# adrientremblay/Skillshot_Learning

Hardware: AMD Instinct MI355X
Metric: env-steps/sec (whole node) at 65536 self-play envs; 1/2/4/8 GPU scaling (higher is better)
Workload: dtype f64

## Files before the change

skillshot_learning_amd/csrc/sk_engine.hip:

```cpp
#include <hip/hip_runtime.h>

#include <cmath>
#include <cstdio>
#include <cstdlib>
#include <cstring>
#include <string>
#include <type_traits>
#include <vector>

#include "sk_device.hpp"
#include "sk_host.hpp"
#include "sk_range.hpp"
#include "sk_step.hpp"


using namespace sk;

struct sk_env {
  int32_t n;
  int64_t env_offset;
  uint64_t seed;
  int32_t device;
  sk_config cfg;
  Cfg dcfg;
  View view;
  sk_state_view hview;
  bool owned;
  char* d_aux;
  sk_counters* d_counters;
  uint64_t* d_step;
  int parity;
  int step_variant;
  int multi_policy;
  int multi_split;
  int multi_early;
  int multi_block;
  int multi_stagger;
  int multi_prefetch;
  int multi_pack;
  int multi_fast;
  char* d_pack;
  skh::Host* host;
};

static thread_local std::string g_err;

static int fail(int code, const std::string& msg) {
  g_err = msg;
  return code;
}

#define HIP_TRY(expr)                                                                 \
  do {                                                                                \
    hipError_t _e = (expr);                                                           \
    if (_e != hipSuccess)                                                             \
      return fail(SK_EHIP, std::string(#expr) + ": " + hipGetErrorString(_e));       \
  } while (0)

static constexpr int kBlock = 256;
static constexpr int64_t kFastStepMinEnvs = 196608;
static constexpr int64_t kFastStepMaxEnvs = 786432;
static constexpr int64_t kSplitStepMaxEnvs = 8192;
static constexpr int64_t kEarlyDrawMinEnvs = 32768;
constexpr int64_t kPackMinEnvs = 65536;
static constexpr int64_t kSplitMultiMaxEnvs = 32768;
static constexpr int64_t kSplitPackMinEnvs = 40960;
static constexpr int64_t kSplitPackMaxEnvs = 98304;
static constexpr int kFastSplitMinTicks = 100;
static constexpr int kSteadyRest = 7;
static inline int64_t counter_slots(int64_t n) {
  const int64_t w2 = (2 * n + 63) / 64, w8 = (n + 7) / 8, waves = w2 > w8 ? w2 : w8;
  return waves * SK_CTR_STRIDE > SK_COUNTER_SLOTS ? waves * SK_CTR_STRIDE : SK_COUNTER_SLOTS;
}
static inline size_t aux_bytes(int64_t n) { return 256 + (size_t)counter_slots(n) * sizeof(sk_counters); }

static inline unsigned grid_for(int64_t n) { return (unsigned)((n + kBlock - 1) / kBlock); }
static inline unsigned step_grid(int64_t n) { return (unsigned)((n + kStepBlock - 1) / kStepBlock); }

__device__ __forceinline__ float reward_of(const Cfg& c, const Env& e, int p, int kind, double path_dist) {
  if (kind == SK_REWARD_SIMPLE) {
    int o = 1 - p;
    double mine = dist_point_point(e.qx[p], e.qy[p], e.px[o], e.py[o]);
    double theirs = dist_point_point(e.qx[o], e.qy[o], e.px[p], e.py[p]);
    return (float)(mine - theirs);
  }
  return (float)(-path_dist / (double)c.W);
}

#ifdef SK_TRACE_STEP
__device__ unsigned long long* sk_step_trace;
#define SK_TS(var) const unsigned long long var = __builtin_amdgcn_s_memrealtime()
#else
#define SK_TS(var)
#endif

template <bool OBS>
__global__ void __launch_bounds__(kStepBlock) k_step(StepArgs a, Cfg c) {
  int64_t i = (int64_t)blockIdx.x * kStepBlock + threadIdx.x;
  SK_TS(ts0);
  WaveCtr wc = ctr_load(a.ctr);
  const uint64_t step = step_read(a.step);
  step_advance(a.step, step, 1);
  bool in = i < a.n;
  bool d = false;
  Env e;
  double q_old0 = 0.0, q_old1 = 0.0;
  sktrig::SinCos tq0 = {0.0, 1.0}, tq1 = {0.0, 1.0};
  U4 ru = {0u, 0u, 0u, 0u};
#ifdef SK_TRACE_STEP
  unsigned long long ts1 = 0, ts2 = 0;
#endif
  if (in) {
    load_env(a.v, i, e);
    q_old0 = e.qrot[0];
    q_old1 = e.qrot[1];
    __builtin_amdgcn_sched_barrier(0);
    const float2 a0 = load_action(a.actions + i);
    const float2 a1 = load_action(a.actions + a.n + i);
    __builtin_amdgcn_sched_barrier(0);
    if (a.random_positions && a.n >= kEarlyDrawMinEnvs) {
      ru = draw4(a.seed, (uint64_t)(a.env_offset + i), step, 1u);
      asm volatile("" : "+v"(ru.x), "+v"(ru.y), "+v"(ru.z), "+v"(ru.w));
    }
    __builtin_amdgcn_sched_barrier(0);
#ifdef SK_TRACE_STEP
    __builtin_amdgcn_s_waitcnt(0);
    ts1 = __builtin_amdgcn_s_memrealtime();
    __builtin_amdgcn_sched_barrier(0);
#endif
    bool k0, k1;
    const sktrig::SinCos m0 = sktrig::sincos_bf(e.rot[0], &k0);
    const sktrig::SinCos m1 = sktrig::sincos_bf(e.rot[1], &k1);
    tick_env_m(c, e, m0, m1, k0 & k1, (double)a0.x, (double)a0.y, (double)a1.x, (double)a1.y, OBS ? &tq0 : nullptr,
               OBS ? &tq1 : nullptr);
#ifdef SK_TRACE_STEP
    __builtin_amdgcn_sched_barrier(0);
    ts2 = __builtin_amdgcn_s_memrealtime();
    __builtin_amdgcn_sched_barrier(0);
#endif
  }
  ctr_settle(wc);
  float o0[12], o1[12];
  unsigned amb = 0;
  double g0 = 0.0, g1 = 0.0;
  if (in) {
    if (OBS && (a.obs || a.reward || a.obs_reset)) {
      float pd0, pd1;
      amb = obs_env_sc(c, e, tq0, tq1, o0, o1, &pd0, &pd1, &g0, &g1);
      if (a.obs) {
        store_obs(a.obs, a.n, 0, i, o0);
        store_obs(a.obs, a.n, 1, i, o1);
        if (amb) fix_future_flags_g(c, e, amb, g0, g1, a.obs, a.n, i);
      }
      if (a.reward) {
        a.reward[i] = reward_of(c, e, 0, a.reward_kind, (double)pd0);
        a.reward[a.n + i] = reward_of(c, e, 1, a.reward_kind, (double)pd1);
      }
    }
    d = (!e.live) || (e.ticks >= a.tick_limit);
    if (a.done) a.done[i] = (uint8_t)d;
    if (a.winner) a.winner[i] = (uint8_t)e.winner;
  }
  const int fin_winner = in ? e.winner : 0, fin_ticks = in ? e.ticks : 0;
  if (in && d && a.auto_reset) {
    if (a.random_positions) {
      if (a.n >= kEarlyDrawMinEnvs) reset_random_u(c, e, ru);
      else reset_random(c, e, a.seed, (uint64_t)(a.env_offset + i), step);
    }
    else reset_fixed(c, e);
  }
  if (OBS && in && a.obs_reset) {
    if (d && a.auto_reset) {
      float pd0, pd1;
      amb = obs_env_sc(c, e, sktrig::SinCos{0.0, 1.0}, sktrig::SinCos{0.0, 1.0}, o0, o1, &pd0, &pd1);
    }
    store_obs(a.obs_reset, a.n, 0, i, o0);
    store_obs(a.obs_reset, a.n, 1, i, o1);
    if (amb) fix_future_flags_g(c, e, amb, g0, g1, a.obs_reset, a.n, i);
  }
  if (in) store_env_q(a.v, i, e, q_old0, q_old1);
  if (a.ctr) wave_count(a.ctr, wc, d, fin_winner, fin_ticks);
  if (!in) return;
#ifdef SK_TRACE_STEP
  __builtin_amdgcn_s_waitcnt(0);
  const unsigned long long ts3 = __builtin_amdgcn_s_memrealtime();
  if ((threadIdx.x & 63) == 0 && sk_step_trace) {
    const unsigned waves = gridDim.x * (blockDim.x >> 6);
    const unsigned w = blockIdx.x * (blockDim.x >> 6) + (threadIdx.x >> 6);
    unsigned long long* t = sk_step_trace + ((step & 15) * waves + w) * 8;
    t[0] = ts0; t[1] = ts1; t[2] = ts2; t[3] = ts3;
    t[4] = __builtin_amdgcn_s_getreg((31 << 11) | 4);
    t[5] = __builtin_amdgcn_s_getreg((15 << 11) | 20);
  }
#endif
}

#ifdef SK_TRACE_STEP
extern "C" int skdiag_set_step_trace(void* buf) {
  return hipMemcpyToSymbol(HIP_SYMBOL(sk_step_trace), &buf, sizeof(buf)) == hipSuccess ? 0 : -1;
}
#endif

__global__ void __launch_bounds__(kStepBlock) k_step_fast(StepArgs a, Cfg c) {
  int64_t i = (int64_t)blockIdx.x * kStepBlock + threadIdx.x;
  bool in = i < a.n;
  StepLoads L;
  if (in) issue_step_loads(a.v, a.actions, a.n, i, L);
  WaveCtr wc = ctr_load(a.ctr);
  bool d = false;
  Env e;
  if (in) {
    wait_rot(L);
    bool k0, k1, k2, k3;
    sktrig::SinCosF m0 = sktrig::sincos_fast(L.r.x, &k0);
    sktrig::SinCosF m1 = sktrig::sincos_fast(L.r.y, &k1);
    wait_qrot(L, m0, m1);
    sktrig::SinCosF tq0 = sktrig::sincos_fast(L.qr.x, &k2);
    sktrig::SinCosF tq1 = sktrig::sincos_fast(L.qr.y, &k3);
    wait_state(L, tq0, tq1);
    decode_env(step_loads_env(L), e);
    wait_actions(L);
    tick_env_fast(c, e, m0, m1, tq0, tq1, k0 & k1, k2, k3, L.a0.x, L.a0.y, L.a1.x, L.a1.y);
// ... 499 lines not shown
      SK_MTW(t, 0);
      asm volatile("s_waitcnt vmcnt(0)" ::: "memory");
      SK_MTW(t, 1);
    }
#endif
    multi_compute<POL, PACK>(a, c, r, rp, L, wc, so, step0, t, w, packed, t + 1 == a.n_ticks, tc);
#if defined(SK_TRACE_MULTI_WAIT)
    SK_MTW(t, 4);
#elif defined(SK_TRACE_MULTI)
    if (t < 29) SK_MTS(1 + t);
#endif
    slab = slab + 1 == a.ring ? 0 : slab + 1;
    pslab = pslab + 1 == a.ring ? 0 : pslab + 1;
    so = so + 1 == a.out_slabs ? 0 : so + 1;
  };
  do {
    one_tick(pa0, pa1);
    if (++t >= a.n_ticks) break;
    one_tick(pa1, pa0);
  } while (++t < a.n_ticks);
  if (a.ctr) {
    const unsigned c4[4] = {L.n_done, L.n_h1, L.n_h2, L.t_sum};
    uint64_t v[4];
    wave_sum4_u32(c4, v);
    ctr_store<BLK>(a.ctr, wc, v[0], v[1], v[2], v[3]);
  }
  step_advance(a.step, step0, (uint64_t)a.n_ticks);
  SK_MTS(31);
}

template <int POL>
__device__ __forceinline__ void st_half_d(const MultiArgs& a, __amdgpu_buffer_rsrc_t r, int k, double* plane, int64_t h,
                                          double v) {
  if constexpr (POL == 0) plane[h] = v;
  else __builtin_amdgcn_raw_buffer_store_b64(__builtin_bit_cast(skb2i, v), r, (uint32_t)h * 8u + a.off[k], 0, 16);
}
template <int POL>
__device__ __forceinline__ void st_half_i(const MultiArgs& a, __amdgpu_buffer_rsrc_t r, int k, int2* plane, int64_t h,
                                          int x, int y) {
  if constexpr (POL == 0) plane[h] = make_int2(x, y);
  else __builtin_amdgcn_raw_buffer_store_b64((skb2i){x, y}, r, (uint32_t)h * 8u + a.off[k], 0, 16);
}
struct SplitLane {
  int64_t i, ic, hc, h;
  int p;
  bool in;
  unsigned n_done, n_h1, n_h2, t_sum;
};

struct SplitCarry {
  double kr, kq;
  sktrig::SinCos m, tq;
  double pr;
  bool qs, have, pend;
};
__device__ __forceinline__ void split_carry_advance(SplitCarry& t) {
  bool k;
  t.m = sktrig::sincos_bf(t.pr, &k);
  if (!k) t.m = sincos_lib(t.pr);
  t.kr = t.pr;
  if (t.qs) {
    t.tq = t.m;
    t.kq = t.pr;
  }
  t.have = true;
  t.pend = false;
}
struct SplitCarryF {
  double kr, kq;
  sktrig::SinCosF m;
  int dx, dy;
  double pr;
  bool mok, qex, have, pend;
};
__device__ __forceinline__ void split_carry_advance(SplitCarryF& t) {
  t.m = sktrig::sincos_fast(t.pr, &t.mok);
  t.kr = t.pr;
  t.have = true;
  t.pend = false;
}
__device__ __forceinline__ void split_carry_pin(SplitCarry& t) {
  asm volatile("" : "+v"(t.m.s), "+v"(t.m.c), "+v"(t.tq.s), "+v"(t.tq.c));
}
__device__ __forceinline__ void split_carry_pin(SplitCarryF& t) {
  asm volatile("" : "+v"(t.m.s), "+v"(t.m.c));
}
template <bool FAST>
struct SplitCarrySel {
  using type = SplitCarry;
};
template <>
struct SplitCarrySel<true> {
  using type = SplitCarryF;
};
struct SplitRaw {
  skb2i rot, qrot, pp, ca, qq, mi;
};
template <int POL>
__device__ __forceinline__ skb2i ld_half_raw(const MultiArgs& a, __amdgpu_buffer_rsrc_t r, int k, const void* plane,
                                             int64_t h) {
  if constexpr (POL == 0) return reinterpret_cast<const skb2i*>(plane)[h];
  else return __builtin_amdgcn_raw_buffer_load_b64(r, (uint32_t)h * 8u + a.off[k], 0, 16);
}
template <int POL>
__device__ __forceinline__ void split_load_raw(const MultiArgs& a, __amdgpu_buffer_rsrc_t r, const SplitLane& L,
                                               SplitRaw& w) {
  w.rot = ld_half_raw<POL>(a, r, 1, a.v.rot, L.hc);
  w.qrot = ld_half_raw<POL>(a, r, 3, a.v.qrot, L.hc);
  w.pp = ld_half_raw<POL>(a, r, 0, a.v.pos, L.hc);
  w.ca = ld_half_raw<POL>(a, r, 4, a.v.qcdage, L.hc);
  w.qq = ld_half_raw<POL>(a, r, 2, a.v.qpos, L.hc);
  w.mi = ld_half_raw<POL>(a, r, 5, a.v.misc, L.ic);
  __builtin_amdgcn_sched_barrier(0);
}
template <int POL>
__device__ __forceinline__ void split_store_state(const MultiArgs& a, __amdgpu_buffer_rsrc_t r, const SplitLane& L,
                                                  int px, int py, double rot, int qx, int qy, double qrot, bool qch,
                                                  int qcd, int qage, int ticks, unsigned f) {
  st_half_i<POL>(a, r, 0, reinterpret_cast<int2*>(a.v.pos), L.h, px, py);
  st_half_d<POL>(a, r, 1, reinterpret_cast<double*>(a.v.rot), L.h, rot);
  st_half_i<POL>(a, r, 2, reinterpret_cast<int2*>(a.v.qpos), L.h, qx, qy);
  if (qch) st_half_d<POL>(a, r, 3, reinterpret_cast<double*>(a.v.qrot), L.h, qrot);
  st_half_i<POL>(a, r, 4, reinterpret_cast<int2*>(a.v.qcdage), L.h, qcd, qage);
  if (L.p == 0) st_half_i<POL>(a, r, 5, a.v.misc, L.i, ticks, (int)f);
}
template <int POL>
__device__ __forceinline__ void split_load_pack(const MultiArgs& a, __amdgpu_buffer_rsrc_t rp, const SplitLane& L,
                                                SplitRaw& w) {
  if constexpr (POL == 0) {
    const skb2i* P = reinterpret_cast<const skb2i*>(a.pack);
    w.rot = P[L.hc];
    w.qrot = P[2 * a.n + L.hc];
    w.pp = P[4 * a.n + L.hc];
  } else {
    const uint32_t o = (uint32_t)L.hc * 8u, plane = (uint32_t)a.n * 16u;
    w.rot = __builtin_amdgcn_raw_buffer_load_b64(rp, o, 0, 16);
    w.qrot = __builtin_amdgcn_raw_buffer_load_b64(rp, o + plane, 0, 16);
    w.pp = __builtin_amdgcn_raw_buffer_load_b64(rp, o + 2u * plane, 0, 16);
  }
  __builtin_amdgcn_sched_barrier(0);
}
template <int POL>
__device__ __forceinline__ void split_store_pack(const MultiArgs& a, __amdgpu_buffer_rsrc_t rp, const SplitLane& L,
                                                 double rot, double qrot, bool store_q, int pos, int cah) {
  if constexpr (POL == 0) {
    skb2i* P = reinterpret_cast<skb2i*>(a.pack);
    P[L.h] = __builtin_bit_cast(skb2i, rot);
    if (store_q) P[2 * a.n + L.h] = __builtin_bit_cast(skb2i, qrot);
    P[4 * a.n + L.h] = (skb2i){pos, cah};
  } else {
    const uint32_t o = (uint32_t)L.h * 8u, plane = (uint32_t)a.n * 16u;
    __builtin_amdgcn_raw_buffer_store_b64(__builtin_bit_cast(skb2i, rot), rp, o, 0, 16);
    if (store_q) __builtin_amdgcn_raw_buffer_store_b64(__builtin_bit_cast(skb2i, qrot), rp, o + plane, 0, 16);
    __builtin_amdgcn_raw_buffer_store_b64((skb2i){pos, cah}, rp, o + 2u * plane, 0, 16);
  }
}
struct SplitSteady {
  __amdgpu_buffer_rsrc_t ra, rd, rw;
  uint32_t va, vd;
  uint32_t aso, dso;
};
struct SplitPre {
  float l;
  double dl;
  sktrig::SinCosF u;
  float ex, ey;
  float mdx, mdy;
  bool msafe, qsafe;
  int imx, imy, iex, iey;
};
__device__ __forceinline__ SplitPre split_fast_pre(const sktrig::SinCosF& m, bool mok, float2 act, const Cfg& c) {
  SplitPre q;
  const float qsf = (float)c.qspeed;
  q.l = clamp_action_f(act.y);
  q.dl = (double)q.l * c.look;
  q.u = sktrig::sincos_add(m, q.l * (float)c.look);
  q.ex = q.u.s * qsf;
  q.ey = q.u.c * qsf;
  const sktrig::FastDelta dm = sktrig::fast_move_delta(m, mok, (float)c.pspeed, clamp_action_f(act.x));
  q.mdx = dm.x;
  q.mdy = dm.y;
  q.msafe = dm.safe;
  q.qsafe = sktrig::fast_step_delta(q.u, mok, qsf).safe;
  q.imx = (int)rintf(q.mdx);
  q.imy = (int)rintf(q.mdy);
  q.iex = (int)rintf(q.ex);
  q.iey = (int)rintf(q.ey);
  return q;
}
__device__ __forceinline__ void split_pre_pin(SplitPre& q) {
  unsigned long long ms = __builtin_amdgcn_ballot_w64(q.msafe), qs = __builtin_amdgcn_ballot_w64(q.qsafe);
  asm volatile("" : "+v"(q.dl), "+v"(q.imx), "+v"(q.imy), "+v"(q.iex), "+v"(q.iey), "+s"(ms), "+s"(qs));
  q.msafe = __builtin_amdgcn_inverse_ballot_w64(ms);
  q.qsafe = __builtin_amdgcn_inverse_ballot_w64(qs);
}
template <int POL, bool OBS, bool PACK = false, bool FAST = false, bool STEADY = false, bool FULL = false>
__device__ __forceinline__ void split_tick_carry(const MultiArgs& a, const Cfg& c, __amdgpu_buffer_rsrc_t r,
                                                 SplitLane& L, WaveCtr& wc, int64_t so, uint64_t step,
                                                 const SplitRaw& w, float2 act,
                                                 typename SplitCarrySel<FAST>::type& tc, bool last,
                                                 __amdgpu_buffer_rsrc_t rp, bool& packed,
                                                 const SplitSteady* ss = nullptr, SplitPre* pre = nullptr,
                                                 int left = 0, bool* admit = nullptr) {
  constexpr bool PRE = FAST && STEADY;
  static_assert(!(OBS && PACK), "the full contract never packs");
  static_assert(!(OBS && FAST), "the observation needs the exact sincos");
  static_assert(PACK || !STEADY, "the steady loop is the packed kernel's");
  static_assert(STEADY || !FULL, "the full-wave form is the steady loop's");
  using sktrig::round_safe;
  const int p = L.p;
  const bool in = FULL || L.in;
  double rot = __builtin_bit_cast(double, w.rot), qrot = __builtin_bit_cast(double, w.qrot);
  int px = w.pp.x, py = w.pp.y, qx = w.qq.x, qy = w.qq.y, qcd = w.ca.x, qage = w.ca.y, ticks = w.mi.x;
  const unsigned flags = (unsigned)w.mi.y;
  int qvalid = (flags >> (8 * p)) & 0xff, live = (flags >> 16) & 0xff, winner = (flags >> 24) & 0xff;
  if constexpr (PACK) {
    if (STEADY || packed) {
      const unsigned s = (unsigned)w.pp.x, ch = (unsigned)w.pp.y;
      px = s & 0xff; py = (s >> 8) & 0xff; qx = (s >> 16) & 0xff; qy = s >> 24;
      qcd = (int)(signed char)(ch & 0xff); qage = (ch >> 8) & 0xff;
      const unsigned hi = ch >> 16, ohi = (unsigned)pair_swap((int)hi);
      const unsigned fl = p ? hi : ohi;
      ticks = (int)(p ? ohi : hi);
      qvalid = (fl >> p) & 1; live = (fl >> 2) & 1; winner = (fl >> 3) & 3;
    }
  }
  const double q_old = qrot;
  const bool f = qcd <= 0;
  const bool miss = (!STEADY && !tc.have) || !same_bits(rot, tc.kr) || (qvalid && !f && !same_bits(qrot, tc.kq));
  if (__ballot(in && miss) != 0) {
    if constexpr (FAST) {
      bool kq;
      tc.m = sktrig::sincos_fast(rot, &tc.mok);
      const sktrig::SinCosF q = sktrig::sincos_fast(qrot, &kq);
      const sktrig::FastDelta d = sktrig::fast_step_delta(q, kq, (float)c.qspeed);
      tc.qex = !d.safe;
      tc.dx = (int)rintf(d.x);
      tc.dy = (int)rintf(d.y);
    } else {
      bool k0, k1;
      tc.m = sktrig::sincos_bf(rot, &k0);
      tc.tq = sktrig::sincos_bf(qrot, &k1);
      if (!(k0 & k1)) {
        if (!k0) tc.m = sincos_lib(rot);
        if (!k1) tc.tq = sincos_lib(qrot);
      }
    }
    tc.kr = rot;
    tc.kq = qrot;
    tc.have = true;
    if constexpr (PRE) *pre = split_fast_pre(tc.m, tc.mok, act, c);
  }
  SplitPre q{};
  if constexpr (PRE) q = *pre;
  const float l = PRE ? q.l : clamp_action_f(act.y);
  const double rn = rot + (PRE ? q.dl : (double)l * c.look);
  const float lk = (float)c.look, qsf = (float)c.qspeed, eq = 2e-6f * qsf;
  sktrig::SinCosF mf;
  if constexpr (FAST) mf = tc.m;
  else mf = sktrig::SinCosF{(float)tc.m.s, (float)tc.m.c};
  const sktrig::SinCosF u = PRE ? q.u : sktrig::sincos_add(mf, l * lk);
  const float ex = PRE ? q.ex : u.s * qsf, ey = PRE ? q.ey : u.c * qsf;
  bool un, unq = false;
  float mdx = 0.0f, mdy = 0.0f;
  sktrig::SinCos tt{0.0, 1.0};
  sktrig::SinCos tm{0.0, 1.0};
  if constexpr (PRE) {
    mdx = q.mdx;
    mdy = q.mdy;
    unq = f && !q.qsafe;
    un = !q.msafe || unq || (qvalid && !f && tc.qex);
  } else if constexpr (FAST) {
    const sktrig::FastDelta dm = sktrig::fast_move_delta(tc.m, tc.mok, (float)c.pspeed, clamp_action_f(act.x));
    mdx = dm.x;
    mdy = dm.y;
    unq = f && !sktrig::fast_step_delta(u, tc.mok, qsf).safe;
    un = !dm.safe || unq || (qvalid && !f && tc.qex);
  } else {
    un = f && !((int)(fabs(rot) < 1647099.3291652855) & (int)round_safe(ex, eq) & (int)round_safe(ey, eq));
    tt = tc.tq;
    tm = tc.m;
  }
  bool fast = f;
  bool exact = false;
  int epx = 0, epy = 0, enx = 0, eny = 0;
  sktrig::SinCos xn{0.0, 1.0};
  sktrig::SinCosF pr{0.0f, 1.0f};
  if constexpr (OBS) {
    bool kx, k2;
    xn = sktrig::sincos_bf(rn, &kx);
    pr = sktrig::sincos_fast(rn, &k2);
    if (!(kx & k2)) {
      if (!kx) xn = sincos_lib(rn);
      if (!k2) {
        const sktrig::SinCos rr = sincos_lib(rn);
        pr.s = (float)rr.s;
        pr.c = (float)rr.c;
      }
    }
  }
  if (__builtin_expect(__ballot(in && un) != 0, 0)) {
    if constexpr (FAST) {
      const double qa = f ? rn : qrot;
      bool k0, k1;
      tm = sktrig::sincos_bf(rot, &k0);
      tt = sktrig::sincos_bf(qa, &k1);
      if (!(k0 & k1)) {
        if (!k0) tm = sincos_lib(rot);
        if (!k1) tt = sincos_lib(qa);
      }
      const double speed = clamp_action((double)act.x), psp = (double)c.pspeed, qsp = (double)c.qspeed;
      const double nxf = __builtin_rint((double)px - (tm.s * psp) * speed);
      const double nyf = __builtin_rint((double)py - (tm.c * psp) * speed);
      const bool ok = (nxf >= 0.0) & (nxf + (double)c.psize <= (double)c.W) & (nyf >= 0.0) &
                      (nyf + (double)c.psize <= (double)c.H);
      epx = ok ? (int)(ok ? nxf : 0.0) : px;
      epy = ok ? (int)(ok ? nyf : 0.0) : py;
      enx = (int)__builtin_rint((double)(f ? epx : qx) - tt.s * qsp);
      eny = (int)__builtin_rint((double)(f ? epy : qy) - tt.c * qsp);
      exact = true;
    } else {
      sktrig::SinCos x = xn;
      if constexpr (!OBS) {
        bool k;
        x = sktrig::sincos_bf(rn, &k);
        if (!k) x = sincos_lib(rn);
      }
      if (f) tt = x;
      fast = false;
    }
  }
  sktrig::SinCos tq_obs{0.0, 1.0};
  if constexpr (OBS) tq_obs = f ? xn : tc.tq;
  if constexpr (!FAST) {
    const double speed = clamp_action((double)act.x), psp = (double)c.pspeed;
    const double nxf = __builtin_rint((double)px - (tm.s * psp) * speed);
    const double nyf = __builtin_rint((double)py - (tm.c * psp) * speed);
    const bool ok = (nxf >= 0.0) & (nxf + (double)c.psize <= (double)c.W) & (nyf >= 0.0) &
                    (nyf + (double)c.psize <= (double)c.H);
    px = ok ? (int)(ok ? nxf : 0.0) : px;
    py = ok ? (int)(ok ? nyf : 0.0) : py;
  } else {
    const int nx = px - (PRE ? q.imx : (int)rintf(mdx)), ny = py - (PRE ? q.imy : (int)rintf(mdy));
    bool ok;
    if constexpr (STEADY) ok = skrange::fits_board(nx, ny, c.W - c.psize, c.H - c.psize);
    else ok = (nx >= 0) & (nx <= c.W - c.psize) & (ny >= 0) & (ny <= c.H - c.psize);
    px = exact ? epx : (ok ? nx : px);
    py = exact ? epy : (ok ? ny : py);
  }
  rot = rn;
  qx = f ? px : qx;
  qy = f ? py : qy;
  qrot = f ? rot : qrot;
  qvalid = f ? 1 : qvalid;
  qcd = f ? c.cdmax : qcd;
  qage = f ? 0 : qage;
  const int lv = live != 0;
  ticks += lv;
  {
    const double qsp = (double)c.qspeed;
    int nx, ny;
    if constexpr (FAST) {
      const int sdx = f ? (PRE ? q.iex : (int)rintf(ex)) : tc.dx, sdy = f ? (PRE ? q.iey : (int)rintf(ey)) : tc.dy;
      tc.dx = sdx;
      tc.dy = sdy;
      tc.qex = f ? unq : tc.qex;
      tc.kq = f ? rn : tc.kq;
      nx = exact ? enx : qx - sdx;
      ny = exact ? eny : qy - sdy;
    } else {
      const int nxF = qx - (int)rintf(ex), nyF = qy - (int)rintf(ey);
      const int nxE = (int)__builtin_rint((double)qx - tt.s * qsp), nyE = (int)__builtin_rint((double)qy - tt.c * qsp);
      nx = fast ? nxF : nxE;
      ny = fast ? nyF : nyE;
    }
    bool ok;
    if constexpr (STEADY) ok = skrange::fits_board(nx, ny, c.W - c.qsize, c.H - c.qsize);
    else ok = (nx + c.qsize <= c.W) & (nx >= 0) & (ny + c.qsize <= c.H) & (ny >= 0);
    const bool upd = lv && qvalid;
    qx = (upd && ok) ? nx : qx;
    qy = (upd && ok) ? ny : qy;
    qvalid = (upd && !ok) ? 0 : qvalid;
    qcd -= lv;
    qage += lv;
  }
  int opx = 0, opy = 0;
  if constexpr (!PACK) {
    opx = pair_swap(px);
    opy = pair_swap(py);
  }
  const int oqx = pair_swap(qx), oqy = pair_swap(qy), oqv = pair_swap(qvalid);
  if constexpr (PACK) {
    bool mine;
    if constexpr (STEADY) mine = (int)(oqv != 0) & (int)skrange::box_hit(px, py, c.psize, oqx, oqy, c.qsize);
    else mine = hit_test_s(c, px, py, oqx, oqy, oqv);
    const bool theirs = pair_swap((int)mine) != 0;
    const skrange::PairHit h = skrange::pair_hit(lv != 0, p ? theirs : mine, p ? mine : theirs);
    winner = h.h1 ? 1 : (h.h2 ? 2 : winner);
    live = ((int)h.h1 | (int)h.h2) ? 0 : live;
  } else {
    const int p1x = p ? opx : px, p1y = p ? opy : py, q1x = p ? oqx : qx, q1y = p ? oqy : qy, q1v = p ? oqv : qvalid;
    const int p2x = p ? px : opx, p2y = p ? py : opy, q2x = p ? qx : oqx, q2y = p ? qy : oqy, q2v = p ? qvalid : oqv;
    const bool h1 = lv && hit_test_s(c, p1x, p1y, q2x, q2y, q2v);
    const bool h2 = lv && !h1 && hit_test_s(c, p2x, p2y, q1x, q1y, q1v);
    winner = h1 ? 1 : (h2 ? 2 : winner);
    live = (h1 || h2) ? 0 : live;
  }
  if constexpr (!STEADY) ctr_settle(wc);
  bool to_pack = STEADY;
  if constexpr (PACK && !STEADY) {
    const bool fit = !in || ((int)pack_fits_player(px, py, qx, qy, qcd, qage, qvalid) &
                               (int)pack_fits_game(ticks, live, winner));
    to_pack = !last && __ballot(!fit) == 0;
    const bool adm = !in || ((int)skrange::admit_player(px, py, qx, qy, qcd, qage, qvalid) &
                               (int)skrange::admit_game(ticks, live, winner, left));
    *admit = to_pack && __ballot(!adm) == 0;
  }
  if (PACK && to_pack) {
    const bool qch = (!STEADY && !packed) || __double_as_longlong(qrot) != __double_as_longlong(q_old);
    const unsigned hi = p ? pack_flags(oqv, qvalid, live, winner) : (unsigned)ticks;
    if (in) split_store_pack<POL>(a, rp, L, rot, qrot, qch, pack_pos(px, py, qx, qy), pack_cah(qcd, qage, hi));
  } else {
    const unsigned fl = (unsigned)(qvalid & 0xff) | ((unsigned)(oqv & 0xff) << 8) | ((unsigned)(live & 0xff) << 16) |
                        ((unsigned)(winner & 0xff) << 24);
    const bool qch = STEADY || (PACK && packed) || __double_as_longlong(qrot) != __double_as_longlong(q_old);
    if (in) split_store_state<POL>(a, r, L, px, py, rot, qx, qy, qrot, qch, qcd, qage, ticks, fl);
  }
  bool amb = false;
  double gq = 0.0;
  const int aqx = qx, aqy = qy;
  const double aqrot = qrot;
  if constexpr (OBS) {
    if (in) {
      float o[12], pd;
      obs12_sc(c, px, py, rot, pr, qx, qy, qrot, tq_obs, qcd, qvalid, opx, opy, o, &pd, &amb, &gq);
      if (a.obs) store_obs(a.obs + so * 24 * a.n, a.n, p, L.i, o);
      if (a.reward) {
        float rw;
        if (a.reward_kind == SK_REWARD_SIMPLE) {
          const double mine = dist_point_point(qx, qy, opx, opy);
          const double theirs = dist_point_point(oqx, oqy, px, py);
          rw = (float)(mine - theirs);
        } else {
          rw = (float)(-(double)pd / (double)c.W);
        }
        a.reward[so * 2 * a.n + (int64_t)p * a.n + L.i] = rw;
      }
    }
  }
  const bool d = in && ((!live) || (ticks >= a.tick_limit));
  if (in && p == 0) {
    if constexpr (STEADY) {
      __builtin_amdgcn_raw_buffer_store_b8((unsigned char)d, ss->rd, ss->vd, ss->dso, 0);
      __builtin_amdgcn_raw_buffer_store_b8((unsigned char)winner, ss->rw, ss->vd, ss->dso, 0);
    } else {
      if (a.done) a.done[so * a.out_stride + L.i] = (uint8_t)d;
      if (a.winner) a.winner[so * a.out_stride + L.i] = (uint8_t)winner;
    }
  }
  bool any_done = true, rs = false;
  if constexpr (STEADY) any_done = __ballot(d) != 0;
  if (any_done) {
    const bool dc = d && p == 0;
    L.n_done += dc;
    L.n_h1 += dc && winner == 1;
    L.n_h2 += dc && winner == 2;
    L.t_sum += dc ? (unsigned)ticks : 0u;
    rs = d && a.auto_reset;
    if (rs) {
      if (a.random_positions) {
        const U4 u4 = draw4(a.seed, (uint64_t)(a.env_offset + L.i), step, 1u);
        px = u32_to_pos(p ? u4.z : u4.x, c.rlo, c.rhi);
        py = u32_to_pos(p ? u4.w : u4.y, c.rlo, c.rhi);
      } else {
        px = p ? c.f2x : c.f1x;
        py = p ? c.f2y : c.f1y;
      }
      rot = 0.0; qx = 0; qy = 0; qrot = 0.0; qcd = 0; qage = 0; qvalid = 0;
      ticks = 0; live = 1; winner = 0;
    }
    const int ov = pair_swap(qvalid);
    if (PACK && to_pack) {
      const unsigned hi = p ? pack_flags(ov, qvalid, live, winner) : (unsigned)ticks;
      if (rs) split_store_pack<POL>(a, rp, L, rot, qrot, true, pack_pos(px, py, qx, qy), pack_cah(qcd, qage, hi));
    } else if (rs) {
      const unsigned fl = (unsigned)(qvalid & 0xff) | ((unsigned)(ov & 0xff) << 8) | ((unsigned)(live & 0xff) << 16) |
                          ((unsigned)(winner & 0xff) << 24);
      split_store_state<POL>(a, r, L, px, py, rot, qx, qy, qrot, true, qcd, qage, ticks, fl);
    }
  }
  if constexpr (PACK) packed = to_pack;
  if constexpr (OBS) {
    if (amb && a.obs) {
      const int fi = future_flag_interval(c, aqx, aqy, opx, opy, gq);
      const float fv = fi >= 0 ? (float)fi : future_flag_cr(c, aqx, aqy, aqrot, opx, opy);
      a.obs[so * 24 * a.n + ((int64_t)p * a.n + L.i) * 12 + 11] = fv;
    }
    tc.m = rs ? sktrig::SinCos{0.0, 1.0} : xn;
    tc.kr = rot;
    tc.tq = tq_obs;
    tc.kq = qrot;
    tc.have = true;
  } else if (STEADY || !last) {
    tc.pr = rot;
    if constexpr (!FAST) tc.qs = same_bits(qrot, rot);
    tc.pend = true;
  }
}

template <int POL, int BLK, bool OBS = false, int PF = 0, bool PACK = false, bool FAST = false>
__global__ void __launch_bounds__(BLK + (PF > 0 ? 64 : 0)) k_step_split_multi(MultiArgs a, Cfg c, int stagger) {
  if constexpr (PF > 0) {
    __shared__ int4 pf_scratch[64];
    if (threadIdx.x >= BLK) {
      prefetch_wave<BLK / 2, PF>(a, pf_scratch);
      return;
    }
  }
  SplitLane L;
  const int64_t gt = (int64_t)blockIdx.x * BLK + threadIdx.x;
  L.i = gt >> 1;
  L.p = (int)(gt & 1);
  L.in = L.i < a.n;
  L.ic = L.in ? L.i : 0;
  L.hc = 2 * L.ic + L.p;
  L.h = 2 * L.i + L.p;
  L.n_done = L.n_h1 = L.n_h2 = L.t_sum = 0;
  if (stagger > 0 && (threadIdx.x >> 6) >= (BLK >> 7))
    for (int k = 0; k < stagger; ++k) __builtin_amdgcn_s_sleep(8);
  WaveCtr wc = ctr_load<BLK>(a.ctr);
  const uint64_t step0 = step_read(a.step);
  step_advance(a.step, step0, (uint64_t)a.n_ticks);
  const __amdgpu_buffer_rsrc_t r = raw_rsrc(a.base), rp = PACK ? raw_rsrc(a.pack) : r;
  bool packed = false;
  bool admitted = false;
  int64_t slab = a.slab0, so = a.out0;
  const int64_t aoff = (int64_t)L.p * a.n + L.ic;
  float2 pa0 = load_action(a.actions + slab * 2 * a.n + aoff), pa1;
  int64_t pslab = slab + 1 == a.ring ? 0 : slab + 1;
  typename SplitCarrySel<FAST>::type tc;
  tc.have = tc.pend = false;
  int t = 0;
  auto one_tick = [&](const float2& cur, float2& nxt) {
    SplitRaw w;
    if constexpr (PF > 0) __builtin_amdgcn_s_barrier();
    if (PACK && packed) split_load_pack<POL>(a, rp, L, w);
    else split_load_raw<POL>(a, r, L, w);
    const int64_t ls = t + 1 < a.n_ticks ? pslab : slab;
    nxt = load_action(a.actions + ls * 2 * a.n + aoff);
    __builtin_amdgcn_sched_barrier(0);
    if (tc.pend) split_carry_advance(tc);
    __builtin_amdgcn_sched_barrier(0);
    if constexpr (PACK)
      split_tick_carry<POL, OBS, PACK, FAST>(a, c, r, L, wc, so, step0 + (uint64_t)t, w, cur, tc, t + 1 == a.n_ticks,
                                             rp, packed, nullptr, nullptr, a.n_ticks - 1 - t, &admitted);
    else
      split_tick_carry<POL, OBS, PACK, FAST>(a, c, r, L, wc, so, step0 + (uint64_t)t, w, cur, tc, t + 1 == a.n_ticks,
                                             rp, packed);
    slab = slab + 1 == a.ring ? 0 : slab + 1;
    pslab = pslab + 1 == a.ring ? 0 : pslab + 1;
    so = so + 1 == a.out_slabs ? 0 : so + 1;
  };
  if constexpr (PACK) {
    SplitSteady S;
    const uint32_t slab_b = (uint32_t)a.n * 16u, ring_b = (uint32_t)a.ring * slab_b;
    const uint32_t out_b = (uint32_t)a.out_slabs * (uint32_t)a.out_stride;
    S.ra = __builtin_amdgcn_make_buffer_rsrc(const_cast<float2*>(a.actions), (short)0, (int)ring_b, 0x00020000);
    S.rd = __builtin_amdgcn_make_buffer_rsrc(a.done, (short)0, __builtin_amdgcn_readfirstlane(a.done ? -1 : 0),
                                             0x00020000);
    S.rw = __builtin_amdgcn_make_buffer_rsrc(a.winner, (short)0, __builtin_amdgcn_readfirstlane(a.winner ? -1 : 0),
                                             0x00020000);
    S.va = (uint32_t)aoff * 8u;
    S.vd = (uint32_t)L.ic;
    S.aso = S.dso = 0;
    const bool full_wave = __ballot(L.in) == ~0ull;
    auto steady_tick = [&](auto full, const float2& cur, float2& nxt) __attribute__((always_inline)) {
      SplitRaw w;
      split_load_pack<POL>(a, rp, L, w);
      const skb2i na = __builtin_amdgcn_raw_buffer_load_b64(S.ra, S.va, S.aso, 2);
      nxt = make_float2(__int_as_float(na.x), __int_as_float(na.y));
      __builtin_amdgcn_sched_barrier(0);
      split_carry_advance(tc);
      split_carry_pin(tc);
      SplitPre pre{};
      if constexpr (FAST) {
        pre = split_fast_pre(tc.m, tc.mok, cur, c);
        split_pre_pin(pre);
      }
      __builtin_amdgcn_sched_barrier(0);
      split_tick_carry<POL, false, true, FAST, true, decltype(full)::value>(a, c, r, L, wc, 0, step0 + (uint64_t)t, w,
                                                                            cur, tc, false, rp, packed, &S, &pre);
      if constexpr (FAST) __builtin_amdgcn_s_sleep(kSteadyRest);
      S.aso = S.aso + slab_b == ring_b ? 0u : S.aso + slab_b;
      S.dso = S.dso + (uint32_t)a.out_stride == out_b ? 0u : S.dso + (uint32_t)a.out_stride;
    };
    do {
      one_tick(pa0, pa1);
      if (++t >= a.n_ticks) break;
      if (a.steady32 && admitted && t + 2 < a.n_ticks) {
        const int t_in = t;
        const uint32_t slab_in = (uint32_t)slab, so_in = (uint32_t)so;
        S.aso = (uint32_t)pslab * slab_b;
        S.dso = so_in * (uint32_t)a.out_stride;
        float2 sa0 = pa0, sa1 = pa1;
        asm volatile("" : "+v"(sa1.x), "+v"(sa1.y));
        auto steady_turns = [&](auto full) __attribute__((always_inline)) {
          do {
            steady_tick(full, sa1, sa0);
            ++t;
            steady_tick(full, sa0, sa1);
            ++t;
          } while (t + 2 < a.n_ticks);
        };
        if (full_wave) steady_turns(std::true_type{});
        else steady_turns(std::false_type{});
        pa0 = sa0;
        pa1 = sa1;
        asm volatile("" : "+v"(pa0.x), "+v"(pa0.y), "+v"(pa1.x), "+v"(pa1.y));
        const uint32_t dt = (uint32_t)(t - t_in);
        slab = (int64_t)((slab_in + dt) % (uint32_t)a.ring);
        pslab = slab + 1 == a.ring ? 0 : slab + 1;
        so = (int64_t)((so_in + dt) % (uint32_t)a.out_slabs);
      }
      one_tick(pa1, pa0);
    } while (++t < a.n_ticks);
  } else {
    do {
      one_tick(pa0, pa1);
      if (++t >= a.n_ticks) break;
      one_tick(pa1, pa0);
    } while (++t < a.n_ticks);
  }
  if (a.ctr) {
    const unsigned c4[4] = {L.n_done, L.n_h1, L.n_h2, L.t_sum};
    uint64_t v[4];
    wave_sum4_u32(c4, v);
    ctr_store<BLK>(a.ctr, wc, v[0], v[1], v[2], v[3]);
  }
}

__global__ void __launch_bounds__(kBlock) k_gen_actions(float4* out, int64_t n, int n_ticks, uint64_t seed,
                                                        int64_t env_offset, StepRef sref) {
  const uint64_t step0 = step_read(sref);
  int64_t i = (int64_t)blockIdx.x * kBlock + threadIdx.x;
  if (i >= n) return;
  float2* o = reinterpret_cast<float2*>(out);
  for (int t = 0; t < n_ticks; ++t) {
    U4 u = draw4(seed, (uint64_t)(env_offset + i), step0 + (uint64_t)t, 0u);
    o[(int64_t)t * 2 * n + i] = make_float2(u32_to_action(u.x), u32_to_action(u.y));
    o[(int64_t)t * 2 * n + n + i] = make_float2(u32_to_action(u.z), u32_to_action(u.w));
  }
}

__global__ void __launch_bounds__(kBlock) k_reset(View v, int64_t n, const uint8_t* mask, int random,
                                                  uint64_t seed, int64_t env_offset, StepRef sref, Cfg c) {
  int64_t i = (int64_t)blockIdx.x * kBlock + threadIdx.x;
  const uint64_t step = step_read(sref);
  step_advance(sref, step, 1);
  if (i >= n || (mask && !mask[i])) return;
  Env e;
  if (random) reset_random(c, e, seed, (uint64_t)(env_offset + i), step);
  else reset_fixed(c, e);
  store_env(v, i, e);
}

__global__ void __launch_bounds__(kBlock) k_move_direction(View v, int64_t n, int p, const double* vals,
                                                           double scalar, Cfg c) {
  int64_t i = (int64_t)blockIdx.x * kBlock + threadIdx.x;
  if (i >= n) return;
  Env e;
  load_env(v, i, e);
  double x = vals ? vals[i] : scalar;
  if (p == 0) move_direction(c, e, 0, x); else move_direction(c, e, 1, x);
  store_env(v, i, e);
}

__global__ void __launch_bounds__(kBlock) k_move_look(View v, int64_t n, int p, const double* vals,
                                                      double scalar, Cfg c) {
  int64_t i = (int64_t)blockIdx.x * kBlock + threadIdx.x;
  if (i >= n) return;
  Env e;
  load_env(v, i, e);
  double x = vals ? vals[i] : scalar;
  if (p == 0) move_look(c, e, 0, x); else move_look(c, e, 1, x);
  store_env(v, i, e);
}

__global__ void __launch_bounds__(kBlock) k_move_discrete(View v, int64_t n, int p, int kind,
                                                          const uint8_t* mask, Cfg c) {
  int64_t i = (int64_t)blockIdx.x * kBlock + threadIdx.x;
  if (i >= n || (mask && !mask[i])) return;
  Env e;
  load_env(v, i, e);
  if (kind == 0) { if (p == 0) move_fwd_back(c, e, 0, false); else move_fwd_back(c, e, 1, false); }
  else if (kind == 1) { if (p == 0) move_fwd_back(c, e, 0, true); else move_fwd_back(c, e, 1, true); }
  else if (kind == 2) { if (p == 0) e.rot[0] += c.look; else e.rot[1] += c.look; }
  else { if (p == 0) e.rot[0] -= c.look; else e.rot[1] -= c.look; }
  store_env(v, i, e);
}

__global__ void __launch_bounds__(kBlock) k_shoot(View v, int64_t n, int p, const uint8_t* mask, Cfg c) {
  int64_t i = (int64_t)blockIdx.x * kBlock + threadIdx.x;
  if (i >= n || (mask && !mask[i])) return;
  Env e;
  load_env(v, i, e);
  if (p == 0) shoot(c, e, 0); else shoot(c, e, 1);
  store_env(v, i, e);
}

__global__ void __launch_bounds__(kBlock) k_projectile_move(View v, int64_t n, int p, int tick,
                                                            const uint8_t* mask, Cfg c) {
  int64_t i = (int64_t)blockIdx.x * kBlock + threadIdx.x;
  if (i >= n || (mask && !mask[i])) return;
  Env e;
  load_env(v, i, e);
  if (p == 0) projectile_tick_s(c, e.qx[0], e.qy[0], e.qrot[0], e.qcd[0], e.qage[0], e.qvalid[0]);
  else projectile_tick_s(c, e.qx[1], e.qy[1], e.qrot[1], e.qcd[1], e.qage[1], e.qvalid[1]);
  if (!tick) {
    if (p == 0) { e.qcd[0] += 1; e.qage[0] -= 1; } else { e.qcd[1] += 1; e.qage[1] -= 1; }
  }
  store_env(v, i, e);
}

__global__ void __launch_bounds__(kBlock) k_check_collision(View v, int64_t n, uint8_t* hit_out, Cfg c) {
  int64_t i = (int64_t)blockIdx.x * kBlock + threadIdx.x;
  if (i >= n) return;
  Env e;
  load_env(v, i, e);
  int live = e.live, winner = e.winner;
  int hit_live = 1, hit = 0;
  collide_s(c, e.px[0], e.py[0], e.qx[0], e.qy[0], e.qvalid[0], e.px[1], e.py[1], e.qx[1], e.qy[1], e.qvalid[1],
            hit_live, hit);
  if (hit) { winner = hit; live = 0; }
  e.live = live;
  e.winner = winner;
  if (hit_out) hit_out[i] = (uint8_t)hit;
  store_env(v, i, e);
}

__global__ void __launch_bounds__(kBlock) k_game_tick(View v, int64_t n, Cfg c) {
  int64_t i = (int64_t)blockIdx.x * kBlock + threadIdx.x;
  if (i >= n) return;
// ... 1000 lines not shown
```

Measured before the change: 46.63 billion.

## Issue steady pack store early under raised wave priority, shorten sleep

In the steady split tick, the packed-state store now happens right after the qvalid swap instead of after hit testing. The code around it runs at raised wave priority (s_setprio 1), which drops back to 0 once the store is issued. Because the store now precedes hit detection, an extra pack-word store is added for pairs that just ended without a reset, so the live and winner flags still get written. The steady s_sleep drops from 7 to 3. The aim is to get memory traffic out earlier and give the critical section priority, at the cost of an extra conditional store and a possible correctness risk in the flag ordering.

```diff
diff --git a/skillshot_learning_amd/csrc/sk_engine.hip b/skillshot_learning_amd/csrc/sk_engine.hip
--- a/skillshot_learning_amd/csrc/sk_engine.hip
+++ b/skillshot_learning_amd/csrc/sk_engine.hip
@@ -67,7 +67,8 @@
 static constexpr int64_t kSplitPackMinEnvs = 40960;
 static constexpr int64_t kSplitPackMaxEnvs = 98304;
 static constexpr int kFastSplitMinTicks = 100;
-static constexpr int kSteadyRest = 7;
+static constexpr int kSteadyRest = 3;
+static constexpr bool kSteadyPrio = true;
 static inline int64_t counter_slots(int64_t n) {
   const int64_t w2 = (2 * n + 63) / 64, w8 = (n + 7) / 8, waves = w2 > w8 ? w2 : w8;
   return waves * SK_CTR_STRIDE > SK_COUNTER_SLOTS ? waves * SK_CTR_STRIDE : SK_COUNTER_SLOTS;
@@ -873,6 +874,16 @@
     const uint32_t o = (uint32_t)L.h * 8u, plane = (uint32_t)a.n * 16u;
     __builtin_amdgcn_raw_buffer_store_b64(__builtin_bit_cast(skb2i, rot), rp, o, 0, 16);
     if (store_q) __builtin_amdgcn_raw_buffer_store_b64(__builtin_bit_cast(skb2i, qrot), rp, o + plane, 0, 16);
+    __builtin_amdgcn_raw_buffer_store_b64((skb2i){pos, cah}, rp, o + 2u * plane, 0, 16);
+  }
+}
+template <int POL>
+__device__ __forceinline__ void split_store_pack_word(const MultiArgs& a, __amdgpu_buffer_rsrc_t rp,
+                                                      const SplitLane& L, int pos, int cah) {
+  if constexpr (POL == 0) {
+    reinterpret_cast<skb2i*>(a.pack)[4 * a.n + L.h] = (skb2i){pos, cah};
+  } else {
+    const uint32_t o = (uint32_t)L.h * 8u, plane = (uint32_t)a.n * 16u;
     __builtin_amdgcn_raw_buffer_store_b64((skb2i){pos, cah}, rp, o + 2u * plane, 0, 16);
   }
 }
@@ -1110,7 +1121,21 @@
     opx = pair_swap(px);
     opy = pair_swap(py);
   }
-  const int oqx = pair_swap(qx), oqy = pair_swap(qy), oqv = pair_swap(qvalid);
+  int oqx, oqy, oqv;
+  if constexpr (STEADY) {
+    oqv = pair_swap(qvalid);
+    const bool qch = __double_as_longlong(qrot) != __double_as_longlong(q_old);
+    const unsigned hi = p ? pack_flags(oqv, qvalid, live, winner) : (unsigned)ticks;
+    if (in) split_store_pack<POL>(a, rp, L, rot, qrot, qch, pack_pos(px, py, qx, qy), pack_cah(qcd, qage, hi));
+    if constexpr (kSteadyPrio) __builtin_amdgcn_s_setprio(0);
+    __builtin_amdgcn_sched_barrier(0);
+    oqx = pair_swap(qx);
+    oqy = pair_swap(qy);
+  } else {
+    oqx = pair_swap(qx);
+    oqy = pair_swap(qy);
+    oqv = pair_swap(qvalid);
+  }
   if constexpr (PACK) {
     bool mine;
     if constexpr (STEADY) mine = (int)(oqv != 0) & (int)skrange::box_hit(px, py, c.psize, oqx, oqy, c.qsize);
@@ -1137,7 +1162,8 @@
                                (int)skrange::admit_game(ticks, live, winner, left));
     *admit = to_pack && __ballot(!adm) == 0;
   }
-  if (PACK && to_pack) {
+  if constexpr (STEADY) {
+  } else if (PACK && to_pack) {
     const bool qch = (!STEADY && !packed) || __double_as_longlong(qrot) != __double_as_longlong(q_old);
     const unsigned hi = p ? pack_flags(oqv, qvalid, live, winner) : (unsigned)ticks;
     if (in) split_store_pack<POL>(a, rp, L, rot, qrot, qch, pack_pos(px, py, qx, qy), pack_cah(qcd, qage, hi));
@@ -1204,6 +1230,10 @@
     if (PACK && to_pack) {
       const unsigned hi = p ? pack_flags(ov, qvalid, live, winner) : (unsigned)ticks;
       if (rs) split_store_pack<POL>(a, rp, L, rot, qrot, true, pack_pos(px, py, qx, qy), pack_cah(qcd, qage, hi));
+      if constexpr (STEADY) {
+        if (d && !rs && lv && !live && p)
+          split_store_pack_word<POL>(a, rp, L, pack_pos(px, py, qx, qy), pack_cah(qcd, qage, hi));
+      }
     } else if (rs) {
       const unsigned fl = (unsigned)(qvalid & 0xff) | ((unsigned)(ov & 0xff) << 8) | ((unsigned)(live & 0xff) << 16) |
                           ((unsigned)(winner & 0xff) << 24);
@@ -1309,6 +1339,11 @@
         split_pre_pin(pre);
       }
       __builtin_amdgcn_sched_barrier(0);
+      if constexpr (kSteadyPrio) {
+        asm volatile("" : "+v"(w.rot.x), "+v"(w.rot.y), "+v"(w.qrot.x), "+v"(w.qrot.y), "+v"(w.pp.x), "+v"(w.pp.y));
+        __builtin_amdgcn_s_setprio(1);
+        __builtin_amdgcn_sched_barrier(0);
+      }
       split_tick_carry<POL, false, true, FAST, true, decltype(full)::value>(a, c, r, L, wc, 0, step0 + (uint64_t)t, w,
                                                                             cur, tc, false, rp, packed, &S, &pre);
       if constexpr (FAST) __builtin_amdgcn_s_sleep(kSteadyRest);
```

New measurement: 49.56 billion (median of 6 runs). +6.3%, better.
